# apernet/hysteria

Measured on AMD Instinct MI355X. Metric: device-resident packet-obfs GiB/s @ 1200B datagrams, 1/2/4/8 MI355X, higher is better.
Workload: dtype u8; 1 GPU; uniform 1048576 x 1200 B datagrams per GPU (configs[1]), dense slotted output; datagrams_per_gpu=1048576, datagram_len=1200, global_datagrams=1048576, psk=average_password, parallelism=packet-index shards x1

## Files before the change

### hysteria_amd/csrc/salamander.hip

```cpp
#include <unistd.h>

#include <atomic>
#include <chrono>

#include "salamander_flat.h"

namespace hyobfs {

#define HY_EXTERN_SW(n)                                                                                   \
    extern template void launch_wave_sw<true, true, n>(const BatchParams&, const KeyParams&, hipStream_t);  \
    extern template void launch_wave_sw<true, false, n>(const BatchParams&, const KeyParams&, hipStream_t); \
    extern template void launch_wave_sw<false, true, n>(const BatchParams&, const KeyParams&, hipStream_t); \
    extern template void launch_wave_sw<false, false, n>(const BatchParams&, const KeyParams&, hipStream_t); \
    extern template void launch_tile_sw<true, n>(const BatchParams&, const KeyParams&, const TileParams&,   \
                                                 hipStream_t);                                              \
    extern template void launch_tile_sw<false, n>(const BatchParams&, const KeyParams&, const TileParams&,  \
                                                  hipStream_t);                                             \
    extern template void launch_flat_sw<true, n>(const BatchParams&, const KeyParams&, const FlatParams&,   \
                                                 hipStream_t);                                              \
    extern template void launch_flat_sw<false, n>(const BatchParams&, const KeyParams&, const FlatParams&,  \
                                                  hipStream_t);
HY_EXTERN_SW(0) HY_EXTERN_SW(1) HY_EXTERN_SW(2) HY_EXTERN_SW(3) HY_EXTERN_SW(4) HY_EXTERN_SW(5)
HY_EXTERN_SW(6) HY_EXTERN_SW(7) HY_EXTERN_SW(8) HY_EXTERN_SW(9) HY_EXTERN_SW(10) HY_EXTERN_SW(11)
HY_EXTERN_SW(12) HY_EXTERN_SW(13) HY_EXTERN_SW(14) HY_EXTERN_SW(15)
#undef HY_EXTERN_SW

template <bool OBF>
__global__ __launch_bounds__(256) void tile_sums_kernel(BatchParams B, uint64_t ntiles) {
    const uint32_t lane = threadIdx.x & 63;
    const uint64_t tile = (uint64_t)blockIdx.x * 4 + (threadIdx.x >> 6);
    const uint64_t p0 = tile * kTile + 4ull * lane;
    uint64_t sw = 0, sl = 0;
#pragma unroll
    for (int k = 0; k < 4; ++k) {
        if (p0 + k < B.n) {
            const uint32_t L = pkt_len(B, p0 + k);
            sw += out_width<OBF>(L, B.pkt_cap);
            sl += L;
        }
    }
    sw = wave_sum(sw);
    if (B.in_tile_sums) sl = wave_sum(sl);
    if (lane == 0 && tile < ntiles) {
        B.tile_sums[tile] = sw;
        if (B.in_tile_sums) B.in_tile_sums[tile] = sl;
    }
}

__global__ __launch_bounds__(1024) void scan_tiles_kernel(uint64_t* v, uint64_t* v2, uint64_t ntiles,
                                                         uint64_t* init2 = nullptr) {
    constexpr int PER = 8, BLK = 64 * PER;
    constexpr int PAD = PER + 1;
    __shared__ uint64_t s_x[16][64 * PAD];
    __shared__ uint64_t s_w[16];
    __shared__ uint64_t s_carry;
    uint64_t* const arr = blockIdx.x ? v2 : v;
    const int t = threadIdx.x, lane = t & 63, wid = t >> 6;
    if (t == 0) s_carry = 0;
    if (init2 && blockIdx.x == 0 && t < 2) init2[t] = ~0ull;
    __syncthreads();
    for (uint64_t base = 0; base < ntiles; base += 16 * BLK) {
        const uint64_t wb = base + (uint64_t)wid * BLK;
#pragma unroll
        for (int k = 0; k < PER; ++k) {
            const int j = 64 * k + lane;
            const uint64_t i = wb + (uint64_t)j;
            s_x[wid][(j / PER) * PAD + j % PER] = i < ntiles ? arr[i] : 0;
        }
        hy_wave_sync();
        uint64_t* row = &s_x[wid][lane * PAD];
        uint64_t run = 0;
#pragma unroll
        for (int k = 0; k < PER; ++k) {
            const uint64_t x = row[k];
            row[k] = run;
            run += x;
        }
        const uint64_t inc = wave_incl_scan(run, lane);
        if (lane == 63) s_w[wid] = inc;
        __syncthreads();
        uint64_t wpre = 0;
        for (int w = 0; w < wid; ++w) wpre += s_w[w];
        const uint64_t off = s_carry + wpre + inc - run;
#pragma unroll
        for (int k = 0; k < PER; ++k) row[k] += off;
        hy_wave_sync();
#pragma unroll
        for (int k = 0; k < PER; ++k) {
            const int j = 64 * k + lane;
            const uint64_t i = wb + (uint64_t)j;
            if (i < ntiles) arr[i] = s_x[wid][(j / PER) * PAD + j % PER];
        }
        __syncthreads();
        if (t == 0) {
            uint64_t tot = 0;
            for (int w = 0; w < 16; ++w) tot += s_w[w];
            s_carry += tot;
        }
        __syncthreads();
    }
    if (t == 0) arr[ntiles] = s_carry;
}

__global__ __launch_bounds__(256) void in_offsets_kernel(BatchParams B, uint64_t* in_off) {
    const uint32_t lane = threadIdx.x & 63;
    const uint64_t tile = (uint64_t)blockIdx.x * 4 + (threadIdx.x >> 6);
    if (tile * kTile >= B.n) return;
    const uint64_t p0 = tile * kTile + 4ull * lane;
    uint32_t L[4];
    uint64_t sl = 0;
#pragma unroll
    for (int k = 0; k < 4; ++k) {
        L[k] = p0 + k < B.n ? B.in_len[p0 + k] : 0u;
        sl += L[k];
    }
    uint64_t x = B.in_tile_prefix[tile] + wave_incl_scan(sl, (int)lane) - sl;
#pragma unroll
    for (int k = 0; k < 4; ++k) {
        if (p0 + k < B.n) in_off[p0 + k] = x;
        x += L[k];
    }
}

__global__ __launch_bounds__(256) void keys_kernel(KeyParams K, const uint64_t* salts, uint8_t* keys,
                                                   uint64_t n) {
    const uint64_t i = (uint64_t)blockIdx.x * blockDim.x + threadIdx.x;
    if (i >= n) return;
    uint64_t k[4];
    salamander_key(K, salts[i], k);
#pragma unroll
    for (int w = 0; w < 4; ++w) __builtin_memcpy(keys + 32 * i + 8 * w, &k[w], 8);
}

__device__ __forceinline__ uint64_t sm64_at(uint64_t seed, uint64_t k) {
    uint64_t z = seed + (k + 1) * 0x9e3779b97f4a7c15ull;
    z = (z ^ (z >> 30)) * 0xbf58476d1ce4e5b9ull;
    z = (z ^ (z >> 27)) * 0x94d049bb133111ebull;
    return z ^ (z >> 31);
}

__global__ void synth_stream_kernel(uint8_t* dst, uint64_t nbytes, uint64_t seed, uint64_t start) {
    const uint64_t i = (uint64_t)blockIdx.x * blockDim.x + threadIdx.x;
    const uint64_t b0 = 16 * i;
    if (b0 >= nbytes) return;
    const uint64_t g = start + b0;
    const uint64_t w = g >> 3;
    const uint32_t s = (uint32_t)(g & 7) * 8;
    const uint64_t x0 = sm64_at(seed, w), x1 = sm64_at(seed, w + 1), x2 = sm64_at(seed, w + 2);
    const uint64_t lo = s ? (x0 >> s) | (x1 << (64 - s)) : x0;
    const uint64_t hi = s ? (x1 >> s) | (x2 << (64 - s)) : x1;
    if (b0 + 16 <= nbytes) {
        *reinterpret_cast<uint64_t*>(dst + b0) = lo;
        *reinterpret_cast<uint64_t*>(dst + b0 + 8) = hi;
    } else {
        for (uint64_t j = 0; b0 + j < nbytes; ++j)
            dst[b0 + j] = (uint8_t)((j < 8 ? lo >> (8 * j) : hi >> (8 * (j - 8))));
    }
}

__global__ void synth_u64_kernel(uint64_t* dst, uint64_t n, uint64_t seed, uint64_t first) {
    const uint64_t i = (uint64_t)blockIdx.x * blockDim.x + threadIdx.x;
    if (i < n) dst[i] = sm64_at(seed, first + i);
}

__global__ void synth_bimodal_kernel(uint32_t* dst, uint64_t n, uint64_t seed, uint64_t first) {
    const uint64_t i = (uint64_t)blockIdx.x * blockDim.x + threadIdx.x;
    if (i < n) dst[i] = (sm64_at(seed, first + i) % 5) < 2 ? 64u : 1350u;
}


static int kernel_override() {
    static const int v = [] {
        const char* e = std::getenv("HYOBFS_KERNEL");
        return !e                        ? kKernelAuto
               : std::strcmp(e, "wave") == 0 ? kKernelWave
               : std::strcmp(e, "tile") == 0 ? kKernelTile
               : std::strcmp(e, "flat") == 0 ? kKernelFlat
                                             : kKernelAuto;
    }();
    return v;
}

int resolve_kernel(int ctx_kernel) { return ctx_kernel ? ctx_kernel : kernel_override(); }

template <bool OBF, bool PACKED>
static void launch_main(const BatchParams& bp, const KeyParams& k, hipStream_t s) {
    const int kc = resolve_kernel(bp.kernel);
    TileParams T;
    if (!PACKED && kc != kKernelWave && tile_params<OBF>(bp, T)) {
        switch (k.salt_pos >> 3) {
#define HY_CASE(n) \
    case n: launch_tile_sw<OBF, n>(bp, k, T, s); break;
            HY_CASE(0) HY_CASE(1) HY_CASE(2) HY_CASE(3) HY_CASE(4) HY_CASE(5) HY_CASE(6) HY_CASE(7)
            HY_CASE(8) HY_CASE(9) HY_CASE(10) HY_CASE(11) HY_CASE(12) HY_CASE(13) HY_CASE(14)
            HY_CASE(15)
#undef HY_CASE
        }
        return;
    }
    switch (k.salt_pos >> 3) {
#define HY_CASE(n) \
    case n: launch_wave_sw<OBF, PACKED, n>(bp, k, s); break;
        HY_CASE(0) HY_CASE(1) HY_CASE(2) HY_CASE(3) HY_CASE(4) HY_CASE(5) HY_CASE(6) HY_CASE(7)
        HY_CASE(8) HY_CASE(9) HY_CASE(10) HY_CASE(11) HY_CASE(12) HY_CASE(13) HY_CASE(14)
        HY_CASE(15)
#undef HY_CASE
    }
}

static uint64_t next_epoch() {
    static std::atomic<uint64_t> ctr{[] {
        const uint64_t t = (uint64_t)std::chrono::steady_clock::now().time_since_epoch().count();
        return (t * 0x9e3779b97f4a7c15ull) ^ ((uint64_t)getpid() << 40);
    }()};
    uint64_t e;
    do e = ctr.fetch_add(1, std::memory_order_relaxed) + 1; while (e == 0);
    return e;
}

static bool flat_eligible(const BatchParams& b) {
    return contiguous_input(b) && b.out_stride == 0 && resolve_kernel(b.kernel) == kKernelFlat &&
           (reinterpret_cast<uintptr_t>(b.in) & 15u) == 0;
}
static bool wave_scans_input(const BatchParams& b) {
    return contiguous_input(b) && b.out_stride == 0 && !flat_eligible(b) && wave_packed_run_log2() == 6;
}

uint64_t batch_workspace_bytes(bool obf, const BatchParams& b) {
    (void)obf;
    if (b.n == 0) return 0;
    const uint64_t tsums = (div_up(b.n, kTile) + 1) * 8;
    if (!contiguous_input(b)) return b.out_stride == 0 ? tsums : 0;
    if (flat_eligible(b)) return 2 * tsums + flat_workspace_bytes(b.out_cap, b.n);
    return 2 * tsums + (wave_scans_input(b) ? 0 : 8 * b.n);
}

int batch_kernel(bool obf, const BatchParams& b) {
    if (b.n == 0) return kKernelAuto;
    if (flat_eligible(b)) return kKernelFlat;
    TileParams T;
    BatchParams bp = b;
    if (contiguous_input(b) && !wave_scans_input(b))
        bp.in_off = reinterpret_cast<const uint64_t*>(16);
    const bool tile = bp.out_stride != 0 && resolve_kernel(bp.kernel) != kKernelWave &&
                      (obf ? tile_params<true>(bp, T) : tile_params<false>(bp, T));
    return tile ? kKernelTile : kKernelWave;
}

template <bool OBF>
static hipError_t launch_contiguous(BatchParams& bp, const KeyParams& k, hipStream_t s, bool& done) {
    done = false;
    if (!bp.scratch) return hipErrorInvalidValue;
    const uint64_t ntiles = div_up(bp.n, kTile);
    bp.tile_sums = static_cast<uint64_t*>(bp.scratch);
    bp.in_tile_sums = bp.tile_sums + ntiles + 1;
    if (flat_eligible(bp)) {
        FlatParams F;
        F.cut = bp.in_tile_sums + ntiles + 1;
        F.desc = reinterpret_cast<FlatDesc*>(F.cut + 2);
        F.out_total = bp.tile_sums + ntiles;
        F.in_total = bp.in_tile_sums + ntiles;
        F.ntiles_max = flat_ntiles_max(bp.out_cap);
        F.krec = reinterpret_cast<uint8_t*>((reinterpret_cast<uintptr_t>(F.cut) + flat_desc_bytes(bp.out_cap) + 255) &
                                            ~(uintptr_t)255);
        F.epoch = next_epoch();
        F.nhash = flat_hashers();
        const dim3 grid((uint32_t)div_up(ntiles, 4)), block(256);
        hipLaunchKernelGGL(tile_sums_kernel<OBF>, grid, block, 0, s, bp, ntiles);
        hipLaunchKernelGGL(scan_tiles_kernel, dim3(2), dim3(1024), 0, s, bp.tile_sums, bp.in_tile_sums, ntiles, F.cut);
        bp.tile_prefix = bp.tile_sums;
        bp.in_tile_prefix = bp.in_tile_sums;
        hipLaunchKernelGGL(flat_locate_kernel<OBF>, grid, block, 0, s, bp, F, ntiles);
        switch (k.salt_pos >> 3) {
#define HY_CASE(n) \
    case n: launch_flat_sw<OBF, n>(bp, k, F, s); break;
            HY_CASE(0) HY_CASE(1) HY_CASE(2) HY_CASE(3) HY_CASE(4) HY_CASE(5) HY_CASE(6) HY_CASE(7)
            HY_CASE(8) HY_CASE(9) HY_CASE(10) HY_CASE(11) HY_CASE(12) HY_CASE(13) HY_CASE(14)
            HY_CASE(15)
#undef HY_CASE
        }
        done = true;
        return hipGetLastError();
    }
    if (wave_scans_input(bp)) return hipSuccess;
    uint64_t* in_off = bp.in_tile_sums + ntiles + 1;
    const dim3 grid((uint32_t)div_up(ntiles, 4)), block(256);
    hipLaunchKernelGGL(tile_sums_kernel<OBF>, grid, block, 0, s, bp, ntiles);
    hipLaunchKernelGGL(scan_tiles_kernel, dim3(1), dim3(1024), 0, s, bp.in_tile_sums, nullptr, ntiles);
    bp.in_tile_prefix = bp.in_tile_sums;
    hipLaunchKernelGGL(in_offsets_kernel, grid, block, 0, s, bp, in_off);
    bp.in_off = in_off;
    bp.in_tile_sums = nullptr;
    bp.in_tile_prefix = nullptr;
    return hipGetLastError();
}

hipError_t launch_salamander(bool obf, const BatchParams& b, const KeyParams& k, hipStream_t s) {
    if (b.n == 0) return hipSuccess;
    const uint64_t ntiles = div_up(b.n, kTile);
    if (ntiles > 0x7fffffffull) return hipErrorInvalidValue;
    if (k.nblk == 2 && (k.salt_pos >> 3) != 15) return hipErrorInvalidValue;
    BatchParams bp = b;
    if (contiguous_input(b)) {
        bool done = false;
        const hipError_t e = obf ? launch_contiguous<true>(bp, k, s, done) : launch_contiguous<false>(bp, k, s, done);
        if (e != hipSuccess || done) return e;
    }
    if (bp.out_stride == 0) {
        if (!bp.tile_sums) return hipErrorInvalidValue;
        const dim3 grid((uint32_t)div_up(ntiles, 4)), block(256);
        if (obf)
            hipLaunchKernelGGL(tile_sums_kernel<true>, grid, block, 0, s, bp, ntiles);
        else
            hipLaunchKernelGGL(tile_sums_kernel<false>, grid, block, 0, s, bp, ntiles);
        hipLaunchKernelGGL(scan_tiles_kernel, dim3(bp.in_tile_sums ? 2 : 1), dim3(1024), 0, s, bp.tile_sums,
                           bp.in_tile_sums, ntiles);
        bp.tile_prefix = bp.tile_sums;
        bp.in_tile_prefix = bp.in_tile_sums;
        if (obf)
            launch_main<true, true>(bp, k, s);
        else
            launch_main<false, true>(bp, k, s);
    } else {
        if (obf)
            launch_main<true, false>(bp, k, s);
        else
            launch_main<false, false>(bp, k, s);
    }
    return hipGetLastError();
}

hipError_t launch_keys(const KeyParams& k, const uint64_t* salts, uint8_t* keys, uint64_t n,
                       hipStream_t s) {
    if (n == 0) return hipSuccess;
    hipLaunchKernelGGL(keys_kernel, dim3((uint32_t)div_up(n, 256)), dim3(256), 0, s, k, salts, keys, n);
    return hipGetLastError();
}

hipError_t launch_synth_stream(uint8_t* dst, uint64_t nbytes, uint64_t seed, uint64_t start,
                               hipStream_t s) {
    if (nbytes == 0) return hipSuccess;
    hipLaunchKernelGGL(synth_stream_kernel, dim3((uint32_t)div_up(div_up(nbytes, 16), 256)), dim3(256),
                       0, s, dst, nbytes, seed, start);
    return hipGetLastError();
}

hipError_t launch_synth_u64(uint64_t* dst, uint64_t n, uint64_t seed, uint64_t first, hipStream_t s) {
    if (n == 0) return hipSuccess;
    hipLaunchKernelGGL(synth_u64_kernel, dim3((uint32_t)div_up(n, 256)), dim3(256), 0, s, dst, n, seed,
                       first);
    return hipGetLastError();
}

hipError_t launch_synth_bimodal(uint32_t* dst, uint64_t n, uint64_t seed, uint64_t first,
                                hipStream_t s) {
    if (n == 0) return hipSuccess;
    hipLaunchKernelGGL(synth_bimodal_kernel, dim3((uint32_t)div_up(n, 256)), dim3(256), 0, s, dst, n,
                       seed, first);
    return hipGetLastError();
}

}
```

### hysteria_amd/csrc/salamander_flat.h

```cpp
#pragma once
#include "salamander_tile.h"

namespace hyobfs {

#ifndef HY_FLAT_T
#define HY_FLAT_T 16384
#endif
constexpr uint32_t kFT = HY_FLAT_T;
static_assert(kFT % 4096 == 0 && kFT <= 65536, "a tile is four 16-byte chunks per thread");
constexpr uint32_t kFThreads = kFT / 64;
constexpr uint32_t kFWaves = kFThreads / 64;
constexpr int kFU = 4;
constexpr int kFD = 64;
constexpr uint32_t kFGuard = 32;
template <bool OBF>
constexpr uint32_t flat_stage_bytes() { return kFT + (OBF ? 32u : 8u * kFD + 32u); }
#ifndef HY_FLAT_MIN_WAVES
#define HY_FLAT_MIN_WAVES 7
#endif
constexpr uint32_t kFlatOffWin = 1u << 31;
constexpr uint32_t kFlatOffGrid = 1u << 30;
constexpr uint32_t kFlatWMask = kFlatOffGrid - 1u;

struct FlatDesc {
    uint64_t d;
    uint64_t o;
    uint64_t i;
};

struct FlatParams {
    FlatDesc* desc;
    uint64_t* cut;
    uint64_t ntiles_max;
    const uint64_t* in_total;
    const uint64_t* out_total;
    uint8_t* krec;
    uint64_t epoch;
    uint32_t nhash;
};

inline uint64_t flat_ntiles_max(uint64_t out_cap) { return (out_cap + kFT - 1) / kFT; }
constexpr uint64_t kKeyRec = 64;
inline uint64_t flat_desc_bytes(uint64_t out_cap) { return 16 + sizeof(FlatDesc) * (flat_ntiles_max(out_cap) + 1); }
inline uint64_t flat_workspace_bytes(uint64_t out_cap, uint64_t n) {
    return ((flat_desc_bytes(out_cap) + 255) & ~255ull) + 256 + kKeyRec * n;
}

#ifndef HY_FLAT_HASHERS
#define HY_FLAT_HASHERS 256
#endif
#ifndef HY_FLAT_HASH_PRIO
#define HY_FLAT_HASH_PRIO 3
#endif
inline uint32_t flat_hashers() {
    static const uint32_t v = [] {
        const char* e = std::getenv("HYOBFS_FLAT_HASHERS");
        const long x = e ? std::atol(e) : HY_FLAT_HASHERS;
        return (uint32_t)(x < 0 ? 0 : x > 4096 ? 4096 : x);
    }();
    return v;
}

#ifdef HYOBFS_EMULATE
__device__ __forceinline__ void krec_store(uint8_t* blk, uint32_t off, uint64_t w, uint64_t tag) {
    std::memcpy(blk + off, &w, 8);
    std::memcpy(blk + off + 8, &tag, 8);
}
__device__ __forceinline__ void krec_load(const uint8_t* blk, uint32_t off, uint64_t& w, uint64_t& tag) {
    std::memcpy(&w, blk + off, 8);
    std::memcpy(&tag, blk + off + 8, 8);
}
#else
typedef uint32_t krec_v4 __attribute__((ext_vector_type(4)));
__device__ __forceinline__ __amdgpu_buffer_rsrc_t krec_rsrc(const uint8_t* blk) {
    const uint64_t a = uni64(reinterpret_cast<uint64_t>(blk));
    return __builtin_amdgcn_make_buffer_rsrc(reinterpret_cast<void*>(a), 0, (int)(64 * kKeyRec), 0x00020000);
}
__device__ __forceinline__ void krec_store(uint8_t* blk, uint32_t off, uint64_t w, uint64_t tag) {
    krec_v4 v;
    v.x = (uint32_t)w;
    v.y = (uint32_t)(w >> 32);
    v.z = (uint32_t)tag;
    v.w = (uint32_t)(tag >> 32);
    __builtin_amdgcn_raw_buffer_store_b128(v, krec_rsrc(blk), (int)off, 0, 16);
}
__device__ __forceinline__ void krec_load(const uint8_t* blk, uint32_t off, uint64_t& w, uint64_t& tag) {
    const krec_v4 v = __builtin_amdgcn_raw_buffer_load_b128(krec_rsrc(blk), (int)off, 0, 16);
    w = (uint64_t)v.y << 32 | v.x;
    tag = (uint64_t)v.w << 32 | v.z;
}
#endif

template <bool OBF>
__global__ __launch_bounds__(256) void flat_locate_kernel(BatchParams B, FlatParams F, uint64_t ntiles) {
    const uint32_t lane = threadIdx.x & 63;
    const uint64_t tile = (uint64_t)blockIdx.x * 4 + (threadIdx.x >> 6);
    if (tile >= ntiles) return;
    const uint64_t p0 = tile * kTile + 4ull * lane;
    uint32_t L[4], W[4];
    uint64_t sl = 0, sw = 0;
#pragma unroll
    for (int k = 0; k < 4; ++k) {
        L[k] = p0 + k < B.n ? B.in_len[p0 + k] : 0u;
        W[k] = p0 + k < B.n ? out_width<OBF>(L[k], B.pkt_cap) : 0u;
        sl += L[k];
        sw += W[k];
    }
    const uint64_t wave_o = B.tile_prefix[tile];
    uint64_t o = wave_o + wave_incl_scan(sw, (int)lane) - sw;
    uint64_t i = B.in_tile_prefix[tile] + wave_incl_scan(sl, (int)lane) - sl;
    uint64_t cut = ~0ull;
    uint64_t cut_o = 0;
#pragma unroll
    for (int k = 0; k < 4; ++k) {
        const uint64_t p = p0 + k;
        if (p < B.n) {
            const bool fits = W[k] && o + W[k] <= B.out_cap;
            if (B.out_off) B.out_off[p] = o;
            if (B.out_len) B.out_len[p] = fits ? W[k] : 0u;
            if (fits) {
                for (uint64_t t = (o + kFT - 1) / kFT; t * kFT < o + W[k]; ++t) F.desc[t] = FlatDesc{p, o, i};
            } else if (W[k] && cut == ~0ull) {
                cut = p;
                cut_o = o;
            }
        }
        o += W[k];
        i += L[k];
    }
    const unsigned long long m = __ballot(cut != ~0ull);
    if (m && wave_o <= B.out_cap) {
        const int l0 = __builtin_ctzll(m);
        const uint64_t c = __shfl(cut, l0, 64), co = __shfl(cut_o, l0, 64);
        if (lane == 0) {
            F.cut[0] = co;
            F.cut[1] = c;
        }
    }
}

template <bool OBF>
struct FlatLDS {
    uint8_t stage[kFGuard + flat_stage_bytes<OBF>() + kFGuard];
    uint64_t key[kFD][4];
    uint64_t salt[kFD];
    int32_t o[kFD + 1];
    int32_t dlt[kFD];
    uint32_t w[kFD];
};

template <class LDS>
__device__ __forceinline__ u128 flat_stage16(const LDS& S, int32_t q) {
    const int32_t a = q + (int32_t)kFGuard;
    const int32_t b = a & ~15;
    const uint32_t sh = (uint32_t)(a & 15);
    const u128 A = *reinterpret_cast<const u128*>(S.stage + b);
    const u128 C = *reinterpret_cast<const u128*>(S.stage + b + 16);
    return sh ? (A >> (8 * sh)) | (C << (128 - 8 * sh)) : A;
}

template <class LDS>
__device__ __forceinline__ u128 flat_payload16(const LDS& S, const uint8_t* __restrict__ in, uint64_t ws,
                                               uint32_t wlen, uint64_t ip, uint32_t PL, int32_t base, int32_t need) {
    const int64_t pos = (int64_t)ip + base;
    if (pos >= (int64_t)ws - 16 && pos + need <= (int64_t)(ws + wlen)) return flat_stage16(S, (int32_t)(pos - (int64_t)ws));
    const uint8_t* src = in + ip;
    if (PL >= 16) {
        const int32_t w = min(max(base, 0), (int32_t)PL - 16);
        const u128 V = load16u(src + w);
        const int32_t d = w - base;
        return d >= 0 ? (V << (8 * d)) : (V >> (8 * -d));
    }
    u128 X = 0;
    for (int32_t j = max(base, 0); j < min(base + 16, (int32_t)PL); ++j) X |= (u128)src[j] << (8 * (j - base));
    return X;
}

template <bool OBF, class LDS>
__device__ __forceinline__ void flat_contrib(const LDS& S, const uint8_t* __restrict__ in, uint64_t ws,
                                             uint32_t wlen, uint32_t k, int32_t rel, uint32_t kh, u128& r, uint32_t& cov) {
    constexpr int32_t SALT = OBF ? 8 : 0;
    const uint32_t W = S.w[k] & kFlatWMask;
    const int32_t o = S.o[k];
    if (W == 0 || o >= rel + 16 || o + (int32_t)W <= rel) return;
    if (OBF) {
        const int32_t sb = max(o, rel), se = min(o + 8, rel + 16);
        if (sb < se) {
            u128 Sv = (u128)S.salt[k];
            Sv = o >= rel ? (Sv << (8 * (o - rel))) : (Sv >> (8 * (rel - o)));
            r |= Sv & bytemask((uint32_t)(sb - rel), (uint32_t)(se - rel));
            cov |= ((1u << (se - sb)) - 1u) << (sb - rel);
        }
    }
    const int32_t ps = max(o + SALT, rel), pe = min(o + (int32_t)W, rel + 16);
    if (ps < pe) {
        const uint64_t ip = (uint64_t)((int64_t)ws + (int64_t)(o + SALT) + S.dlt[k]);
        const u128 X = flat_payload16(S, in, ws, wlen, ip, W - (uint32_t)SALT, rel - (o + SALT), pe - rel);
        const uint64_t* kw = S.key[k] + 2 * kh;
        const u128 K = (u128)kw[1] << 64 | kw[0];
        r |= (X ^ K) & bytemask((uint32_t)(ps - rel), (uint32_t)(pe - rel));
        cov |= ((1u << (pe - ps)) - 1u) << (ps - rel);
    }
}

__device__ __forceinline__ uint64_t flat_lomask(int32_t b) {
    const uint32_t c = (uint32_t)min(max(b, 0), 8);
    return c ? ~0ull >> (64u - 8u * c) : 0ull;
}
__device__ __forceinline__ uint64_t flat_bfi(uint64_t m, uint64_t x, uint64_t y) { return (m & x) | (~m & y); }

template <bool OBF, int ND, class LDS>
__device__ __forceinline__ bool flat_chunk(const LDS& S, int32_t rel, uint32_t kh, uint32_t m, u128& value) {
    constexpr int32_t SALT = OBF ? 8 : 0;
    uint32_t q = 0;
#pragma unroll
    for (uint32_t s = ND / 2; s; s >>= 1) q = S.o[q + s] <= rel ? q + s : q;
    const int32_t oq = S.o[q];
    const uint32_t wq = S.w[q];
    const int32_t eq = oq + (int32_t)(wq & kFlatWMask);
    const uint32_t q1 = q + 1;
    const int32_t o1 = S.o[q1];
    const uint32_t w1 = q1 < m ? S.w[q1] : 0u;
    const int32_t e1 = o1 + (int32_t)(w1 & kFlatWMask);
    const bool fast = oq <= rel && (wq & (kFlatOffWin | kFlatOffGrid)) == 0 && eq > rel &&
                      (eq >= rel + 16 || (o1 == eq && (w1 & (kFlatOffWin | kFlatOffGrid)) == 0 && e1 >= rel + 16));
    if (!fast) return false;
    const uint64_t* dq = reinterpret_cast<const uint64_t*>(S.stage + (rel + S.dlt[q] + (int32_t)kFGuard));
    const uint64_t xl = dq[0] ^ S.key[q][kh], xh = dq[1] ^ S.key[q][kh + 1];
    if (oq + SALT <= rel && rel + 16 <= eq) {
        value = (u128)xh << 64 | xl;
        return true;
    }
    uint64_t lo = 0, hi = 0;
    const int32_t b1 = oq + SALT - rel, b2 = eq - rel, b3 = b2 + SALT;
    if (eq < rel + 16) {
        const uint64_t* d1 = reinterpret_cast<const uint64_t*>(S.stage + (rel + S.dlt[q1] + (int32_t)kFGuard));
        lo = d1[0] ^ S.key[q1][kh];
        hi = d1[1] ^ S.key[q1][kh + 1];
        if (OBF) {
            const uint64_t s1 = S.salt[q1];
            const uint32_t e8 = 8u * (uint32_t)b2;
            const uint64_t s1l = e8 < 64 ? s1 << e8 : 0ull;
            const uint64_t s1h = e8 < 64 ? s1 >> (64 - e8) : s1 << (e8 - 64);
            lo = flat_bfi(flat_lomask(b3), s1l, lo);
            hi = flat_bfi(flat_lomask(b3 - 8), s1h, hi);
        }
    }
    lo = flat_bfi(flat_lomask(b2), xl, lo);
    hi = flat_bfi(flat_lomask(b2 - 8), xh, hi);
    if (OBF) {
        const uint32_t c8 = 8u * (uint32_t)min(rel - oq, 8);
        const uint64_t sq = c8 < 64 ? S.salt[q] >> c8 : 0ull;
        lo = flat_bfi(flat_lomask(b1), sq, lo);
    }
    value = (u128)hi << 64 | lo;
    return true;
}

template <bool OBF, int SW>
__device__ __forceinline__ void flat_hasher(const BatchParams& B, const KeyParams& K, const FlatParams& F, uint32_t h,
                                            uint32_t wid) {
    const uint32_t lane = threadIdx.x & 63;
    const uint64_t step = (uint64_t)F.nhash * kFWaves;
#ifndef HYOBFS_EMULATE
    __builtin_amdgcn_s_setprio(HY_FLAT_HASH_PRIO);
#endif
    for (uint64_t blk = (uint64_t)h * kFWaves + wid; blk * 64 < B.n; blk += step) {
        const uint64_t k = blk * 64 + lane;
        const bool live = k < B.n;
        uint64_t salt = 0;
        if (OBF) {
            salt = live ? B.salts[k] : 0ull;
        } else {
            const uint64_t g = blk / 4;
            uint64_t pre = 0;
#pragma unroll
            for (int j = 0; j < 3; ++j) {
                const uint64_t q = g * kTile + 64ull * j + lane;
                if (q < blk * 64) pre += B.in_len[q];
            }
            const uint32_t L = live ? B.in_len[k] : 0u;
            const uint64_t i = B.in_tile_prefix[g] + wave_sum(pre) + wave_incl_scan32(L, (int)lane) - L;
            if (L > 8u) salt = load8u(B.in + i);
        }
        uint64_t key[4];
        wave_key<SW>(K, salt, key);
        uint8_t* kb = F.krec + kKeyRec * blk * 64;
        if (live) {
#pragma unroll
            for (int w = 0; w < 4; ++w) krec_store(kb, (uint32_t)(kKeyRec * lane + 16 * w), key[w], F.epoch);
        }
    }
}

template <bool OBF, int SW>
__global__ __launch_bounds__(kFThreads, HY_FLAT_MIN_WAVES) void salamander_flat_kernel(BatchParams B, KeyParams K,
                                                                                  FlatParams F) {
    constexpr int32_t SALT = OBF ? 8 : 0;
    constexpr uint32_t SKIP = OBF ? 0u : 8u;
    __shared__ __attribute__((aligned(16))) FlatLDS<OBF> S;
    const uint32_t wid = uni32(threadIdx.x >> 6);
    const uint8_t* __restrict__ in = B.in;
    if (blockIdx.x < F.nhash) {
        flat_hasher<OBF, SW>(B, K, F, blockIdx.x, wid);
        return;
    }
    const uint64_t t = blockIdx.x - F.nhash;
    const uint64_t E = uni64(min<uint64_t>(F.cut[0], *F.out_total));
    if (t == 0 && threadIdx.x == 0 && B.out_total) atomicAdd(B.out_total, (unsigned long long)E);
    const uint64_t tT = t * kFT;
    if (tT >= E) return;
    const int32_t tl = (int32_t)min<uint64_t>(kFT, E - tT);
    const FlatDesc D0 = F.desc[t];
    const uint64_t d0 = uni64(D0.d), o0 = uni64(D0.o), i0 = uni64(D0.i);
    const uint64_t dend = uni64(tT + kFT < E ? F.desc[t + 1].d + 1 : min<uint64_t>(F.cut[1], B.n));

    const int64_t first = (int64_t)tT - (int64_t)o0 - SALT;
    const uint64_t ws = (i0 + SKIP + (uint64_t)max<int64_t>(first, 0)) & ~15ull;
    const uint64_t in_total = uni64(*F.in_total);
    const uint32_t wlen = (uint32_t)min<uint64_t>(flat_stage_bytes<OBF>(), in_total > ws ? in_total - ws : 0);
    {
        const uint32_t lane = threadIdx.x & 63;
        const uint32_t nfull = wlen >> 4;
        for (uint32_t c = wid; c * 64u < nfull; c += kFWaves) {
            const uint32_t ch = c * 64u + lane;
            if (ch < nfull) glds16(in + ws + 16ull * ch, S.stage + kFGuard + 1024u * c);
        }
        const uint32_t tail = wlen & 15u;
        if (tail && wid == kFWaves - 1 && lane < tail) S.stage[kFGuard + 16u * nfull + lane] = in[ws + 16ull * nfull + lane];
    }

    uint8_t* __restrict__ ob = B.out + tT;
    uint64_t og = o0, ig = i0;
    for (uint64_t g0 = d0; g0 < dend; g0 += kFD) {
        const uint32_t m = (uint32_t)min<uint64_t>((uint64_t)kFD, dend - g0);
        uint32_t tid = threadIdx.x;
#ifndef HYOBFS_EMULATE
        asm volatile("" : "+v"(tid));
#endif
        const uint32_t lane = tid & 63;
        if (wid == 0) {
            const bool live = lane < m;
            const uint64_t p = g0 + lane;
            const uint32_t L = live ? B.in_len[p] : 0u;
            uint64_t salt = live && OBF ? B.salts[p] : 0ull;
            uint8_t* kb = F.krec + kKeyRec * g0;
            uint64_t kw[4], tg[4];
#pragma unroll
            for (int w = 0; w < 4; ++w) {
                kw[w] = tg[w] = 0;
                if (live && F.nhash) krec_load(kb, (uint32_t)(kKeyRec * lane + 16 * w), kw[w], tg[w]);
            }
            uint32_t W = live ? out_width<OBF>(L, B.pkt_cap) : 0u;
            const uint32_t iw = wave_incl_scan32(W, (int)lane);
            const uint32_t il = wave_incl_scan32(L, (int)lane);
            const uint64_t o = og + iw - W, i = ig + il - L;
            og += uni32((uint32_t)__shfl(iw, 63, 64));
            ig += uni32((uint32_t)__shfl(il, 63, 64));
            if (W && o + W > B.out_cap) W = 0;
            const int32_t orel = (int32_t)((int64_t)o - (int64_t)tT);
            const int32_t dlt = (int32_t)((int64_t)(i + SKIP) - (int64_t)ws) - (orel + SALT);
            bool miss = W && (tg[0] != F.epoch || tg[1] != F.epoch || tg[2] != F.epoch || tg[3] != F.epoch);
            const int spins = F.nhash ? 48 : 0;
            for (int spin = 0; spin < spins && __ballot(miss); ++spin) {
#ifndef HYOBFS_EMULATE
                __builtin_amdgcn_s_sleep(8);
#endif
                if (miss) {
                    miss = false;
#pragma unroll
                    for (int w = 0; w < 4; ++w) {
                        krec_load(kb, (uint32_t)(kKeyRec * lane + 16 * w), kw[w], tg[w]);
                        miss |= tg[w] != F.epoch;
                    }
                }
            }
            if (__ballot(miss)) {
                if (!OBF && W) salt = load8u(in + i);
                for (uint32_t k0 = 0; k0 < m; k0 += 16) {
                    const uint32_t k = k0 + (lane >> 2), qi = lane & 3u;
                    const uint64_t x = quad_key<SW>(K, __shfl(salt, (int)(k < 64 ? k : 0), 64), qi);
                    const uint32_t src = 4u * ((lane - k0) & 15u);
#pragma unroll
                    for (int w = 0; w < 4; ++w) {
                        const uint64_t y = __shfl(x, (int)(src + (uint32_t)w), 64);
                        if (miss && lane >= k0 && lane < k0 + 16) kw[w] = y;
                    }
                }
            }
            uint64_t kr[4];
            rotl_key_bytes(kw, ((uint32_t)o + (uint32_t)SALT) & 31u, kr);
            uint32_t fl = 0;
            if (W) {
                const int32_t ps = max(orel + SALT, 0), pe = min(orel + (int32_t)W, (int32_t)kFT);
                if (ps < pe && (ps + dlt < 0 || pe + dlt > (int32_t)wlen)) fl |= kFlatOffWin;
                if (dlt & 7) fl |= kFlatOffGrid;
            }
            S.o[lane] = live ? orel : 0x7FFFFFFF;
            if (lane == 0) S.o[kFD] = 0x7FFFFFFF;
            S.w[lane] = W | fl;
            S.dlt[lane] = dlt;
            S.salt[lane] = salt;
#pragma unroll
            for (int w = 0; w < 4; ++w) S.key[lane][w] = kr[w];
        }
        __syncthreads();

        u128 r[kFU];
        uint32_t gen = 0;
#pragma unroll
        for (int u = 0; u < kFU; ++u) {
            const int32_t rel = 16 * (int32_t)(u * kFThreads + tid);
            r[u] = 0;
            if (rel >= tl) continue;
            if (!flat_chunk<OBF, kFD>(S, rel, 2u * (((uint32_t)rel >> 4) & 1u), m, r[u])) gen |= 1u << u;
        }
#pragma unroll
        for (int u = 0; u < kFU; ++u) {
            const int32_t rel = 16 * (int32_t)(u * kFThreads + tid);
            if (rel < tl && !((gen >> u) & 1u)) store16_stream(ob + rel, r[u]);
        }
        while (gen) {
            const int u = __builtin_ctz(gen);
            gen &= gen - 1;
            const int32_t rel = 16 * (int32_t)(u * kFThreads + tid);
            uint32_t q = 0;
            for (uint32_t s = kFD / 2; s; s >>= 1) q = S.o[q + s] <= rel ? q + s : q;
            u128 v = 0;
            uint32_t cov = 0;
            for (uint32_t k = q; k < m && S.o[k] < rel + 16; ++k)
                flat_contrib<OBF>(S, in, ws, wlen, k, rel, ((uint32_t)rel >> 4) & 1u, v, cov);
            if (cov == 0xFFFFu)
                store16_stream(ob + rel, v);
            else if (cov)
                store_masked(ob + rel, v, cov);
        }
        if (g0 + kFD < dend) __syncthreads();
    }
}

template <bool OBF, int SW>
void launch_flat_sw(const BatchParams& b, const KeyParams& k, const FlatParams& F, hipStream_t s) {
    const uint64_t nt = F.ntiles_max < 1 ? 1 : F.ntiles_max;
    hipLaunchKernelGGL((salamander_flat_kernel<OBF, SW>), dim3((uint32_t)(F.nhash + nt)), dim3(kFThreads), 0, s, b, k,
                       F);
}

}
```

Baseline: 3094 GiB/s.

## Drop side-block key hashers; compute keys across multiple waves per flat tile

Removes the separate hasher blocks that precomputed per-packet keys into an epoch-tagged global workspace, and the spin-wait polling on those records. Key derivation now happens inline, split across four key waves per tile, each handling 16 datagrams. The tile grows to 32 KiB with 512 threads. A new edge pass resolves packet-boundary chunks into LDS park slots so the main pass can store inner and boundary chunks directly. The aim is to avoid global key-record traffic and the polling stalls, at the cost of more LDS, a larger block, an extra barrier and inline hashing on the critical path.

```diff
diff --git a/hysteria_amd/csrc/salamander.hip b/hysteria_amd/csrc/salamander.hip
--- a/hysteria_amd/csrc/salamander.hip
+++ b/hysteria_amd/csrc/salamander.hip
@@ -1,8 +1,3 @@
-#include <unistd.h>
-
-#include <atomic>
-#include <chrono>
-
 #include "salamander_flat.h"
 
 namespace hyobfs {
@@ -208,19 +203,16 @@
     }
 }
 
-static uint64_t next_epoch() {
-    static std::atomic<uint64_t> ctr{[] {
-        const uint64_t t = (uint64_t)std::chrono::steady_clock::now().time_since_epoch().count();
-        return (t * 0x9e3779b97f4a7c15ull) ^ ((uint64_t)getpid() << 40);
-    }()};
-    uint64_t e;
-    do e = ctr.fetch_add(1, std::memory_order_relaxed) + 1; while (e == 0);
-    return e;
-}
-
+#ifndef HY_FLAT_AUTO_MIN
+#define HY_FLAT_AUTO_MIN 0
+#endif
+constexpr uint64_t kFlatAutoMin = HY_FLAT_AUTO_MIN;
+static_assert(kFlatAutoMin == 0 || kFlatAutoMin >= 131072, "AUTO keeps the wave kernel on small batches");
 static bool flat_eligible(const BatchParams& b) {
-    return contiguous_input(b) && b.out_stride == 0 && resolve_kernel(b.kernel) == kKernelFlat &&
-           (reinterpret_cast<uintptr_t>(b.in) & 15u) == 0;
+    const int kc = resolve_kernel(b.kernel);
+    return contiguous_input(b) && b.out_stride == 0 &&
+           (kc == kKernelFlat || (kc == kKernelAuto && kFlatAutoMin != 0 && b.n >= kFlatAutoMin)) &&
+           ((reinterpret_cast<uintptr_t>(b.in) | reinterpret_cast<uintptr_t>(b.out)) & 15u) == 0;
 }
 static bool wave_scans_input(const BatchParams& b) {
     return contiguous_input(b) && b.out_stride == 0 && !flat_eligible(b) && wave_packed_run_log2() == 6;
@@ -261,10 +253,6 @@
         F.out_total = bp.tile_sums + ntiles;
         F.in_total = bp.in_tile_sums + ntiles;
         F.ntiles_max = flat_ntiles_max(bp.out_cap);
-        F.krec = reinterpret_cast<uint8_t*>((reinterpret_cast<uintptr_t>(F.cut) + flat_desc_bytes(bp.out_cap) + 255) &
-                                            ~(uintptr_t)255);
-        F.epoch = next_epoch();
-        F.nhash = flat_hashers();
         const dim3 grid((uint32_t)div_up(ntiles, 4)), block(256);
         hipLaunchKernelGGL(tile_sums_kernel<OBF>, grid, block, 0, s, bp, ntiles);
         hipLaunchKernelGGL(scan_tiles_kernel, dim3(2), dim3(1024), 0, s, bp.tile_sums, bp.in_tile_sums, ntiles, F.cut);
diff --git a/hysteria_amd/csrc/salamander_flat.h b/hysteria_amd/csrc/salamander_flat.h
--- a/hysteria_amd/csrc/salamander_flat.h
+++ b/hysteria_amd/csrc/salamander_flat.h
@@ -4,19 +4,32 @@
 namespace hyobfs {
 
 #ifndef HY_FLAT_T
-#define HY_FLAT_T 16384
+#define HY_FLAT_T 32768
 #endif
 constexpr uint32_t kFT = HY_FLAT_T;
-static_assert(kFT % 4096 == 0 && kFT <= 65536, "a tile is four 16-byte chunks per thread");
+static_assert(kFT % 4096 == 0 && kFT <= 65536 && kFT / 64 <= 1024, "a tile is four 16-byte chunks per thread");
 constexpr uint32_t kFThreads = kFT / 64;
 constexpr uint32_t kFWaves = kFThreads / 64;
 constexpr int kFU = 4;
-constexpr int kFD = 64;
+#ifndef HY_FLAT_KEY_WAVES
+#define HY_FLAT_KEY_WAVES 4
+#endif
+constexpr uint32_t kFKW = HY_FLAT_KEY_WAVES;
+static_assert((kFKW == 1 || kFKW == 2 || kFKW == 4) && kFKW < kFWaves, "key waves: a power of two, not every wave");
+constexpr int kFD = 16 * (int)kFKW;
+constexpr uint32_t kFKeyRows = 2;
+constexpr uint32_t kFPark = 2 * (kFD + 1);
+static_assert(kFPark <= kFThreads, "one edge thread per parked chunk");
+#ifndef HY_FLAT_EDGE_PASS
+#define HY_FLAT_EDGE_PASS 2
+#endif
+template <bool OBF>
+constexpr bool flat_edge_pass() { return HY_FLAT_EDGE_PASS == 1 || (HY_FLAT_EDGE_PASS == 2 && OBF); }
 constexpr uint32_t kFGuard = 32;
 template <bool OBF>
 constexpr uint32_t flat_stage_bytes() { return kFT + (OBF ? 32u : 8u * kFD + 32u); }
 #ifndef HY_FLAT_MIN_WAVES
-#define HY_FLAT_MIN_WAVES 7
+#define HY_FLAT_MIN_WAVES 8
 #endif
 constexpr uint32_t kFlatOffWin = 1u << 31;
 constexpr uint32_t kFlatOffGrid = 1u << 30;
@@ -34,62 +47,15 @@
     uint64_t ntiles_max;
     const uint64_t* in_total;
     const uint64_t* out_total;
-    uint8_t* krec;
-    uint64_t epoch;
-    uint32_t nhash;
 };
 
 inline uint64_t flat_ntiles_max(uint64_t out_cap) { return (out_cap + kFT - 1) / kFT; }
-constexpr uint64_t kKeyRec = 64;
 inline uint64_t flat_desc_bytes(uint64_t out_cap) { return 16 + sizeof(FlatDesc) * (flat_ntiles_max(out_cap) + 1); }
 inline uint64_t flat_workspace_bytes(uint64_t out_cap, uint64_t n) {
-    return ((flat_desc_bytes(out_cap) + 255) & ~255ull) + 256 + kKeyRec * n;
-}
-
-#ifndef HY_FLAT_HASHERS
-#define HY_FLAT_HASHERS 256
-#endif
-#ifndef HY_FLAT_HASH_PRIO
-#define HY_FLAT_HASH_PRIO 3
-#endif
-inline uint32_t flat_hashers() {
-    static const uint32_t v = [] {
-        const char* e = std::getenv("HYOBFS_FLAT_HASHERS");
-        const long x = e ? std::atol(e) : HY_FLAT_HASHERS;
-        return (uint32_t)(x < 0 ? 0 : x > 4096 ? 4096 : x);
-    }();
-    return v;
-}
-
-#ifdef HYOBFS_EMULATE
-__device__ __forceinline__ void krec_store(uint8_t* blk, uint32_t off, uint64_t w, uint64_t tag) {
-    std::memcpy(blk + off, &w, 8);
-    std::memcpy(blk + off + 8, &tag, 8);
-}
-__device__ __forceinline__ void krec_load(const uint8_t* blk, uint32_t off, uint64_t& w, uint64_t& tag) {
-    std::memcpy(&w, blk + off, 8);
-    std::memcpy(&tag, blk + off + 8, 8);
-}
-#else
-typedef uint32_t krec_v4 __attribute__((ext_vector_type(4)));
-__device__ __forceinline__ __amdgpu_buffer_rsrc_t krec_rsrc(const uint8_t* blk) {
-    const uint64_t a = uni64(reinterpret_cast<uint64_t>(blk));
-    return __builtin_amdgcn_make_buffer_rsrc(reinterpret_cast<void*>(a), 0, (int)(64 * kKeyRec), 0x00020000);
-}
-__device__ __forceinline__ void krec_store(uint8_t* blk, uint32_t off, uint64_t w, uint64_t tag) {
-    krec_v4 v;
-    v.x = (uint32_t)w;
-    v.y = (uint32_t)(w >> 32);
-    v.z = (uint32_t)tag;
-    v.w = (uint32_t)(tag >> 32);
-    __builtin_amdgcn_raw_buffer_store_b128(v, krec_rsrc(blk), (int)off, 0, 16);
-}
-__device__ __forceinline__ void krec_load(const uint8_t* blk, uint32_t off, uint64_t& w, uint64_t& tag) {
-    const krec_v4 v = __builtin_amdgcn_raw_buffer_load_b128(krec_rsrc(blk), (int)off, 0, 16);
-    w = (uint64_t)v.y << 32 | v.x;
-    tag = (uint64_t)v.w << 32 | v.z;
-}
-#endif
+    const uint64_t desc16k = 16 + sizeof(FlatDesc) * ((out_cap + 16383) / 16384 + 1);
+    return ((desc16k + 255) & ~255ull) + 256 + 64 * n;
+}
+static_assert(kFT % 16384 == 0, "the descriptor area is sized for 16 KiB tiles: only whole multiples fit it");
 
 template <bool OBF>
 __global__ __launch_bounds__(256) void flat_locate_kernel(BatchParams B, FlatParams F, uint64_t ntiles) {
@@ -142,11 +108,13 @@
 template <bool OBF>
 struct FlatLDS {
     uint8_t stage[kFGuard + flat_stage_bytes<OBF>() + kFGuard];
+    u128 park[kFPark];
     uint64_t key[kFD][4];
     uint64_t salt[kFD];
     int32_t o[kFD + 1];
     int32_t dlt[kFD];
     uint32_t w[kFD];
+    uint32_t pok[kFPark];
 };
 
 template <class LDS>
@@ -203,6 +171,23 @@
     }
 }
 
+template <int ND, class LDS>
+__device__ __forceinline__ uint32_t flat_search(const LDS& S, int32_t rel) {
+    uint32_t q = 0;
+#pragma unroll
+    for (uint32_t s = ND / 2; s; s >>= 1) q = S.o[q + s] <= rel ? q + s : q;
+    return q;
+}
+
+template <bool OBF, int ND, class LDS>
+__device__ __forceinline__ void flat_merge(const LDS& S, const uint8_t* __restrict__ in, uint64_t ws, uint32_t wlen,
+                                           uint32_t m, int32_t rel, u128& v, uint32_t& cov) {
+    v = 0;
+    cov = 0;
+    for (uint32_t k = flat_search<ND>(S, rel); k < m && S.o[k] < rel + 16; ++k)
+        flat_contrib<OBF>(S, in, ws, wlen, k, rel, ((uint32_t)rel >> 4) & 1u, v, cov);
+}
+
 __device__ __forceinline__ uint64_t flat_lomask(int32_t b) {
     const uint32_t c = (uint32_t)min(max(b, 0), 8);
     return c ? ~0ull >> (64u - 8u * c) : 0ull;
@@ -212,9 +197,7 @@
 template <bool OBF, int ND, class LDS>
 __device__ __forceinline__ bool flat_chunk(const LDS& S, int32_t rel, uint32_t kh, uint32_t m, u128& value) {
     constexpr int32_t SALT = OBF ? 8 : 0;
-    uint32_t q = 0;
-#pragma unroll
-    for (uint32_t s = ND / 2; s; s >>= 1) q = S.o[q + s] <= rel ? q + s : q;
+    const uint32_t q = flat_search<ND>(S, rel);
     const int32_t oq = S.o[q];
     const uint32_t wq = S.w[q];
     const int32_t eq = oq + (int32_t)(wq & kFlatWMask);
@@ -258,42 +241,6 @@
 }
 
 template <bool OBF, int SW>
-__device__ __forceinline__ void flat_hasher(const BatchParams& B, const KeyParams& K, const FlatParams& F, uint32_t h,
-                                            uint32_t wid) {
-    const uint32_t lane = threadIdx.x & 63;
-    const uint64_t step = (uint64_t)F.nhash * kFWaves;
-#ifndef HYOBFS_EMULATE
-    __builtin_amdgcn_s_setprio(HY_FLAT_HASH_PRIO);
-#endif
-    for (uint64_t blk = (uint64_t)h * kFWaves + wid; blk * 64 < B.n; blk += step) {
-        const uint64_t k = blk * 64 + lane;
-        const bool live = k < B.n;
-        uint64_t salt = 0;
-        if (OBF) {
-            salt = live ? B.salts[k] : 0ull;
-        } else {
-            const uint64_t g = blk / 4;
-            uint64_t pre = 0;
-#pragma unroll
-            for (int j = 0; j < 3; ++j) {
-                const uint64_t q = g * kTile + 64ull * j + lane;
-                if (q < blk * 64) pre += B.in_len[q];
-            }
-            const uint32_t L = live ? B.in_len[k] : 0u;
-            const uint64_t i = B.in_tile_prefix[g] + wave_sum(pre) + wave_incl_scan32(L, (int)lane) - L;
-            if (L > 8u) salt = load8u(B.in + i);
-        }
-        uint64_t key[4];
-        wave_key<SW>(K, salt, key);
-        uint8_t* kb = F.krec + kKeyRec * blk * 64;
-        if (live) {
-#pragma unroll
-            for (int w = 0; w < 4; ++w) krec_store(kb, (uint32_t)(kKeyRec * lane + 16 * w), key[w], F.epoch);
-        }
-    }
-}
-
-template <bool OBF, int SW>
 __global__ __launch_bounds__(kFThreads, HY_FLAT_MIN_WAVES) void salamander_flat_kernel(BatchParams B, KeyParams K,
                                                                                   FlatParams F) {
     constexpr int32_t SALT = OBF ? 8 : 0;
@@ -301,11 +248,7 @@
     __shared__ __attribute__((aligned(16))) FlatLDS<OBF> S;
     const uint32_t wid = uni32(threadIdx.x >> 6);
     const uint8_t* __restrict__ in = B.in;
-    if (blockIdx.x < F.nhash) {
-        flat_hasher<OBF, SW>(B, K, F, blockIdx.x, wid);
-        return;
-    }
-    const uint64_t t = blockIdx.x - F.nhash;
+    const uint64_t t = blockIdx.x;
     const uint64_t E = uni64(min<uint64_t>(F.cut[0], *F.out_total));
     if (t == 0 && threadIdx.x == 0 && B.out_total) atomicAdd(B.out_total, (unsigned long long)E);
     const uint64_t tT = t * kFT;
@@ -322,7 +265,11 @@
     {
         const uint32_t lane = threadIdx.x & 63;
         const uint32_t nfull = wlen >> 4;
-        for (uint32_t c = wid; c * 64u < nfull; c += kFWaves) {
+        const bool kwv = wid < kFKW;
+        const uint32_t c0 = kwv ? wid : kFKW * kFKeyRows + (wid - kFKW);
+        const uint32_t cs = kwv ? kFKW : kFWaves - kFKW;
+        const uint32_t ce = kwv ? kFKW * kFKeyRows : ~0u;
+        for (uint32_t c = c0; c < ce && c * 64u < nfull; c += cs) {
             const uint32_t ch = c * 64u + lane;
             if (ch < nfull) glds16(in + ws + 16ull * ch, S.stage + kFGuard + 1024u * c);
         }
@@ -339,18 +286,13 @@
         asm volatile("" : "+v"(tid));
 #endif
         const uint32_t lane = tid & 63;
-        if (wid == 0) {
+        if (wid < kFKW) {
+            const uint32_t k0 = 16u * wid;
             const bool live = lane < m;
+            const bool mine = lane >= k0 && lane < k0 + 16u;
             const uint64_t p = g0 + lane;
             const uint32_t L = live ? B.in_len[p] : 0u;
-            uint64_t salt = live && OBF ? B.salts[p] : 0ull;
-            uint8_t* kb = F.krec + kKeyRec * g0;
-            uint64_t kw[4], tg[4];
-#pragma unroll
-            for (int w = 0; w < 4; ++w) {
-                kw[w] = tg[w] = 0;
-                if (live && F.nhash) krec_load(kb, (uint32_t)(kKeyRec * lane + 16 * w), kw[w], tg[w]);
-            }
+            uint64_t salt = live && mine && OBF ? B.salts[p] : 0ull;
             uint32_t W = live ? out_width<OBF>(L, B.pkt_cap) : 0u;
             const uint32_t iw = wave_incl_scan32(W, (int)lane);
             const uint32_t il = wave_incl_scan32(L, (int)lane);
@@ -358,35 +300,15 @@
             og += uni32((uint32_t)__shfl(iw, 63, 64));
             ig += uni32((uint32_t)__shfl(il, 63, 64));
             if (W && o + W > B.out_cap) W = 0;
+            if (!OBF && mine && W) salt = load8u(in + i);
             const int32_t orel = (int32_t)((int64_t)o - (int64_t)tT);
+            const int32_t pend = (int32_t)((int64_t)og - (int64_t)tT);
             const int32_t dlt = (int32_t)((int64_t)(i + SKIP) - (int64_t)ws) - (orel + SALT);
-            bool miss = W && (tg[0] != F.epoch || tg[1] != F.epoch || tg[2] != F.epoch || tg[3] != F.epoch);
-            const int spins = F.nhash ? 48 : 0;
-            for (int spin = 0; spin < spins && __ballot(miss); ++spin) {
-#ifndef HYOBFS_EMULATE
-                __builtin_amdgcn_s_sleep(8);
-#endif
-                if (miss) {
-                    miss = false;
-#pragma unroll
-                    for (int w = 0; w < 4; ++w) {
-                        krec_load(kb, (uint32_t)(kKeyRec * lane + 16 * w), kw[w], tg[w]);
-                        miss |= tg[w] != F.epoch;
-                    }
-                }
-            }
-            if (__ballot(miss)) {
-                if (!OBF && W) salt = load8u(in + i);
-                for (uint32_t k0 = 0; k0 < m; k0 += 16) {
-                    const uint32_t k = k0 + (lane >> 2), qi = lane & 3u;
-                    const uint64_t x = quad_key<SW>(K, __shfl(salt, (int)(k < 64 ? k : 0), 64), qi);
-                    const uint32_t src = 4u * ((lane - k0) & 15u);
-#pragma unroll
-                    for (int w = 0; w < 4; ++w) {
-                        const uint64_t y = __shfl(x, (int)(src + (uint32_t)w), 64);
-                        if (miss && lane >= k0 && lane < k0 + 16) kw[w] = y;
-                    }
-                }
+            uint64_t kw[4] = {0, 0, 0, 0};
+            if (k0 < m) {
+                const uint64_t x = quad_key<SW>(K, __shfl(salt, (int)(k0 + (lane >> 2)), 64), lane & 3u);
+#pragma unroll
+                for (int w = 0; w < 4; ++w) kw[w] = __shfl(x, (int)(4u * (lane & 15u) + (uint32_t)w), 64);
             }
             uint64_t kr[4];
             rotl_key_bytes(kw, ((uint32_t)o + (uint32_t)SALT) & 31u, kr);
@@ -396,40 +318,95 @@
                 if (ps < pe && (ps + dlt < 0 || pe + dlt > (int32_t)wlen)) fl |= kFlatOffWin;
                 if (dlt & 7) fl |= kFlatOffGrid;
             }
-            S.o[lane] = live ? orel : 0x7FFFFFFF;
-            if (lane == 0) S.o[kFD] = 0x7FFFFFFF;
-            S.w[lane] = W | fl;
-            S.dlt[lane] = dlt;
-            S.salt[lane] = salt;
-#pragma unroll
-            for (int w = 0; w < 4; ++w) S.key[lane][w] = kr[w];
+            if (mine) {
+                S.o[lane] = live ? orel : lane == m ? pend : 0x7FFFFFFF;
+                S.w[lane] = W | fl;
+                S.dlt[lane] = dlt;
+                S.salt[lane] = salt;
+#pragma unroll
+                for (int w = 0; w < 4; ++w) S.key[lane][w] = kr[w];
+            }
+            if (wid == 0 && lane == 0) S.o[kFD] = m == (uint32_t)kFD ? pend : 0x7FFFFFFF;
         }
         __syncthreads();
 
         u128 r[kFU];
         uint32_t gen = 0;
-#pragma unroll
-        for (int u = 0; u < kFU; ++u) {
-            const int32_t rel = 16 * (int32_t)(u * kFThreads + tid);
-            r[u] = 0;
-            if (rel >= tl) continue;
-            if (!flat_chunk<OBF, kFD>(S, rel, 2u * (((uint32_t)rel >> 4) & 1u), m, r[u])) gen |= 1u << u;
-        }
-#pragma unroll
-        for (int u = 0; u < kFU; ++u) {
-            const int32_t rel = 16 * (int32_t)(u * kFThreads + tid);
-            if (rel < tl && !((gen >> u) & 1u)) store16_stream(ob + rel, r[u]);
+        if constexpr (flat_edge_pass<OBF>()) {
+            if (tid < kFPark) {
+                const uint32_t k = OBF ? tid >> 1 : tid, e = OBF ? tid & 1u : 0u;
+                const int32_t a = k <= m ? S.o[k] : 0;
+                const int32_t rel = ((a >> 4) + (int32_t)e) * 16;
+                uint32_t ok = 0;
+                if (k <= m && (e == 0 || (OBF && (a & 15) > 8)) && rel >= 0 && rel < tl) {
+                    u128 v;
+                    uint32_t cov;
+                    flat_merge<OBF, kFD>(S, in, ws, wlen, m, rel, v, cov);
+                    if (cov == 0xFFFFu) {
+                        S.park[tid] = v;
+                        ok = 1;
+                    } else if (cov) {
+                        store_masked(ob + rel, v, cov);
+                    }
+                }
+                S.pok[tid] = ok;
+            }
+            hy_lds_barrier();
+
+            const int32_t pbeg = S.o[0] & ~15, pend = S.o[m];
+            uint32_t st = 0;
+#pragma unroll
+            for (int u = 0; u < kFU; ++u) {
+                const int32_t rel = 16 * (int32_t)(u * kFThreads + tid);
+                r[u] = 0;
+                if (rel >= tl || rel < pbeg || rel >= pend) continue;
+                const uint32_t q = flat_search<kFD>(S, rel);
+                const int32_t a = S.o[q], b = S.o[q + 1], c = rel >> 4;
+                const uint32_t wq = S.w[q];
+                const bool inner = a + SALT <= rel && rel + 16 <= a + (int32_t)(wq & kFlatWMask) &&
+                                   (wq & (kFlatOffWin | kFlatOffGrid)) == 0;
+                constexpr int32_t PS = OBF ? 2 : 1;
+                int32_t slot = -1;
+                if (OBF && (a >> 4) + 1 == c && a + 8 > rel) slot = PS * (int32_t)q + 1;
+                if ((a >> 4) == c) slot = PS * (int32_t)q;
+                if ((b >> 4) == c) slot = PS * (int32_t)q + PS;
+                const uint32_t kh = 2u * ((uint32_t)c & 1u);
+                const uint64_t* dq =
+                    reinterpret_cast<const uint64_t*>(S.stage + ((inner ? rel + S.dlt[q] : 0) + (int32_t)kFGuard));
+                const uint64_t xl = dq[0] ^ S.key[q][kh], xh = dq[1] ^ S.key[q][kh + 1];
+                const uint32_t sl = (uint32_t)max(slot, 0);
+                const u128 pv = S.park[sl];
+                const bool pk = S.pok[sl] != 0;
+                r[u] = inner ? (u128)xh << 64 | xl : pv;
+                if (inner || (slot >= 0 && pk)) st |= 1u << u;
+                if (!inner && slot < 0) gen |= 1u << u;
+            }
+#pragma unroll
+            for (int u = 0; u < kFU; ++u) {
+                const int32_t rel = 16 * (int32_t)(u * kFThreads + tid);
+                if ((st >> u) & 1u) store16_stream(ob + rel, r[u]);
+            }
+        } else {
+#pragma unroll
+            for (int u = 0; u < kFU; ++u) {
+                const int32_t rel = 16 * (int32_t)(u * kFThreads + tid);
+                r[u] = 0;
+                if (rel >= tl) continue;
+                if (!flat_chunk<OBF, kFD>(S, rel, 2u * (((uint32_t)rel >> 4) & 1u), m, r[u])) gen |= 1u << u;
+            }
+#pragma unroll
+            for (int u = 0; u < kFU; ++u) {
+                const int32_t rel = 16 * (int32_t)(u * kFThreads + tid);
+                if (rel < tl && !((gen >> u) & 1u)) store16_stream(ob + rel, r[u]);
+            }
         }
         while (gen) {
             const int u = __builtin_ctz(gen);
             gen &= gen - 1;
             const int32_t rel = 16 * (int32_t)(u * kFThreads + tid);
-            uint32_t q = 0;
-            for (uint32_t s = kFD / 2; s; s >>= 1) q = S.o[q + s] <= rel ? q + s : q;
-            u128 v = 0;
-            uint32_t cov = 0;
-            for (uint32_t k = q; k < m && S.o[k] < rel + 16; ++k)
-                flat_contrib<OBF>(S, in, ws, wlen, k, rel, ((uint32_t)rel >> 4) & 1u, v, cov);
+            u128 v;
+            uint32_t cov;
+            flat_merge<OBF, kFD>(S, in, ws, wlen, m, rel, v, cov);
             if (cov == 0xFFFFu)
                 store16_stream(ob + rel, v);
             else if (cov)
@@ -442,8 +419,7 @@
 template <bool OBF, int SW>
 void launch_flat_sw(const BatchParams& b, const KeyParams& k, const FlatParams& F, hipStream_t s) {
     const uint64_t nt = F.ntiles_max < 1 ? 1 : F.ntiles_max;
-    hipLaunchKernelGGL((salamander_flat_kernel<OBF, SW>), dim3((uint32_t)(F.nhash + nt)), dim3(kFThreads), 0, s, b, k,
-                       F);
-}
-
-}
+    hipLaunchKernelGGL((salamander_flat_kernel<OBF, SW>), dim3((uint32_t)nt), dim3(kFThreads), 0, s, b, k, F);
+}
+
+}
```

Result: slower. 3032 GiB/s (-2.0%).
